# seung-lab/crackle

Measured on AMD Instinct MI355X. Metric: voxels/s encode+decode, 1024x1024x512 uint32; bit-exact .ckl bytes, higher is better.
Workload: dtype u32

## Files before the change

crackle_amd/csrc/ckl_trail.hpp:

```cpp
#pragma once

#include "ckl_device.hpp"

namespace ckl {
namespace dev {

constexpr uint32_t kTrailTileShift = 5, kTrailTileDim = 32;
__device__ __forceinline__ uint32_t mt_index(uint32_t mx, uint32_t my, uint32_t mtx2) {
	return (((my >> 1) * mtx2 + (mx >> 1)) << 2) | ((my & 1u) << 1) | (mx & 1u);
}
struct MicroTile {
	uint4 lo, hi;
	uint32_t mx, my;
	__device__ __forceinline__ bool holds(uint32_t x, uint32_t y) const { return (x >> 3) == mx && (y >> 3) == my; }
	__device__ __forceinline__ uint32_t nib(uint32_t x, uint32_t y) const {
		const uint32_t r = y & 7u;
		const uint32_t a0 = (r & 1u) ? lo.y : lo.x, a1 = (r & 1u) ? lo.w : lo.z, a2 = (r & 1u) ? hi.y : hi.x, a3 = (r & 1u) ? hi.w : hi.z;
		const uint32_t b0 = (r & 2u) ? a1 : a0, b1 = (r & 2u) ? a3 : a2;
		return (((r & 4u) ? b1 : b0) >> ((x & 7u) * 4u)) & 15u;
	}
};

enum : uint32_t { TRAIL_ERR_CAPACITY = 1u };
constexpr uint32_t kDartNone = 0xFFFFFFFFu;
constexpr uint32_t kItemSeg = 0u << 30, kItemCtl = 1u << 30, kItemDead = 2u << 30, kItemMask = 3u << 30;

struct TrailArgs {
	const uint4* adjm;
	uint64_t adjm_stride;
	uint32_t mtx2;
	uint32_t tiles_x, tiles_y;
	const uint32_t* planeV;
	const uint32_t* planeH;
	uint32_t row_words;
	uint64_t plane_words;
	uint32_t sx, sy, inv;
	uint32_t sxe, sye;
	uint32_t nverts;
	uint32_t z0;
	const uint32_t* max_steps;
	uint32_t graph_blocks;
	const uint32_t* blk_special;
	const uint32_t* blk_corner;
	const uint64_t* nbase;
	const uint32_t* ncap;
	uint32_t* n_nodes;
	uint32_t* node_vertex;
	uint8_t* node_adj;
	uint32_t* vert2node;
	const uint64_t* cobase;
	const uint32_t* cocap;
	uint32_t* n_corners;
	uint32_t* corner_vertex;
	uint32_t* dart_end;
	uint32_t* dart_len;
	uint32_t* dart_minv;
	uint32_t* dart_minpos;
	uint4* dart_codes;
	uint8_t* dart_inline;
	uint32_t* parent;
	unsigned long long* compmin;
	uint32_t* start_bits;
	uint32_t start_words;
	uint32_t* starts;
	uint32_t* n_starts;
	const uint64_t* ibase;
	const uint32_t* icap;
	uint32_t* items;
	uint32_t* item_off;
	uint32_t* n_items;
	const uint64_t* sbase;
	const uint32_t* scap;
	uint32_t* stack_node;
	uint32_t* stack_item;
	const uint64_t* kbase;
	const uint32_t* kcap;
	uint32_t* chain_node;
	uint32_t* chain_item0;
	uint32_t* chain_off;
	uint32_t* chain_clen;
	uint32_t* n_chains;
	uint32_t* n_raw;
	uint32_t* n_valid;
	const uint64_t* cbase;
	const uint32_t* ccap;
	uint8_t* cp;
	uint32_t* slice_err;
	uint32_t* events;
	uint32_t* n_events;
	uint32_t* seg_len_sum;
	uint32_t* chain_ev0;
	uint32_t* ev_lnd;
	uint32_t* ev_item;
	uint32_t walk_plain;
	uint32_t walk_stack_cap;
	uint32_t walk_no_regs;
	unsigned long long* dbg;
};

__device__ __forceinline__ void mt_load(MicroTile& c, const uint4* adjm, uint32_t x, uint32_t y, uint32_t mtx2) {
	const uint4* p = adjm + static_cast<uint64_t>(mt_index(x >> 3, y >> 3, mtx2)) * 2u;
	c.lo = p[0]; c.hi = p[1];
	c.mx = x >> 3; c.my = y >> 3;
}
__device__ __forceinline__ void trail_step(uint32_t& x, uint32_t& y, uint32_t k) {
	if (k & 2u) y = (k & 1u) ? y - 1u : y + 1u;
	else x = (k & 1u) ? x - 1u : x + 1u;
}
__device__ __forceinline__ uint32_t trail_code(uint32_t k) { return (0x0231u >> (4u * k)) & 3u; }

struct TileRowBits { uint32_t R, L, D, U; };

__device__ __forceinline__ TileRowBits trail_row_bits(
	const uint32_t* __restrict__ pv, const uint32_t* __restrict__ ph, uint32_t row_words,
	uint32_t sx, uint32_t sy, uint32_t tx, uint32_t y, uint32_t inv
) {
	const uint32_t x0 = tx << 5;
	const uint32_t lt_sx = x0 >= sx ? 0u : (sx - x0 >= 32u ? 0xFFFFFFFFu : ((1u << (sx - x0)) - 1u));
	const uint32_t le_sx = x0 > sx ? 0u : (sx - x0 >= 31u ? 0xFFFFFFFFu : ((2u << (sx - x0)) - 1u));
	const uint32_t ge_1 = tx == 0 ? 0xFFFFFFFEu : 0xFFFFFFFFu;
	TileRowBits b = { 0, 0, 0, 0 };
	const bool have_w = tx < row_words;
	if (y >= 1 && y < sy) {
		const uint32_t h = have_w ? ph[static_cast<uint64_t>(y) * row_words + tx] : 0u;
		const uint32_t hp = tx > 0 ? ph[static_cast<uint64_t>(y) * row_words + tx - 1] : 0u;
		b.R = (h ^ inv) & lt_sx;
		b.L = (((h << 1) | (hp >> 31)) ^ inv) & ge_1 & le_sx;
	}
	if (y < sy) b.D = ((have_w ? pv[static_cast<uint64_t>(y) * row_words + tx] : 0u) ^ inv) & ge_1 & lt_sx;
	if (y >= 1 && y <= sy) b.U = ((have_w ? pv[static_cast<uint64_t>(y - 1) * row_words + tx] : 0u) ^ inv) & ge_1 & lt_sx;
	return b;
}
__device__ __forceinline__ uint32_t trail_special_mask(const TileRowBits& b) {
	const uint32_t a1 = b.R ^ b.L, a2 = b.R & b.L, c1 = b.D ^ b.U, c2 = b.D & b.U;
	const uint32_t bit0 = a1 ^ c1, carry = a1 & c1;
	const uint32_t bit1 = a2 ^ c2 ^ carry, bit2 = (a2 & c2) | (carry & (a2 ^ c2));
	const uint32_t deg2 = ~bit0 & bit1 & ~bit2;
	return (b.R | b.L | b.D | b.U) & ~deg2;
}
__device__ __forceinline__ uint32_t trail_corner_mask(const TileRowBits& b) { return b.R & b.D & ~b.L & ~b.U; }
__device__ __forceinline__ uint32_t spread8(uint32_t m) {
	uint32_t x = (m | (m << 12)) & 0x000F000Fu;
	x = (x | (x << 6)) & 0x03030303u;
	x = (x | (x << 3)) & 0x11111111u;
	return x;
}

__device__ __forceinline__ void trail_rows8(
	const uint32_t* __restrict__ pv, const uint32_t* __restrict__ ph, uint32_t row_words,
	uint32_t sx, uint32_t sy, uint32_t tx, uint32_t y0, uint32_t inv, TileRowBits (&b)[8]
) {
#pragma unroll
	for (int k = 0; k < 8; k++) b[k] = TileRowBits{ 0, 0, 0, 0 };
	if (row_words == 0 || sy == 0) return;
	const uint32_t x0 = tx << 5;
	const uint32_t lt_sx = x0 >= sx ? 0u : (sx - x0 >= 32u ? 0xFFFFFFFFu : ((1u << (sx - x0)) - 1u));
	const uint32_t le_sx = x0 > sx ? 0u : (sx - x0 >= 31u ? 0xFFFFFFFFu : ((2u << (sx - x0)) - 1u));
	const uint32_t ge_1 = tx == 0 ? 0xFFFFFFFEu : 0xFFFFFFFFu;
	const bool have_w = tx < row_words;
	const uint32_t txc = have_w ? tx : row_words - 1u, txp = tx > 0 ? min(tx - 1u, row_words - 1u) : 0u;
	uint32_t hw[8], hpw[8], vw[9];
#pragma unroll
	for (uint32_t k = 0; k < 8; k++) {
		const uint64_t row = static_cast<uint64_t>(min(y0 + k, sy - 1u)) * row_words;
		hw[k] = ph[row + txc];
		hpw[k] = ph[row + txp];
	}
#pragma unroll
	for (uint32_t k = 0; k < 9; k++) {
		const uint32_t y = y0 + k;
		vw[k] = pv[static_cast<uint64_t>(min(y > 0 ? y - 1u : 0u, sy - 1u)) * row_words + txc];
	}
#pragma unroll
	for (uint32_t k = 0; k < 8; k++) {
		const uint32_t y = y0 + k;
		const uint32_t h = have_w ? hw[k] : 0u, hp = tx > 0 ? hpw[k] : 0u;
		if (y >= 1 && y < sy) {
			b[k].R = (h ^ inv) & lt_sx;
			b[k].L = (((h << 1) | (hp >> 31)) ^ inv) & ge_1 & le_sx;
		}
		if (y < sy) b[k].D = ((have_w ? vw[k + 1] : 0u) ^ inv) & ge_1 & lt_sx;
		if (y >= 1 && y <= sy) b[k].U = ((have_w ? vw[k] : 0u) ^ inv) & ge_1 & lt_sx;
	}
}

static __global__ void __launch_bounds__(kBlock) k_trail_graph(
	const uint32_t* __restrict__ planeV, const uint32_t* __restrict__ planeH, uint32_t row_words, uint64_t plane_words,
	uint32_t sx, uint32_t sy, uint32_t perm_mode, const unsigned long long* __restrict__ total_pairs, unsigned long long half_voxels,
	uint32_t* __restrict__ adjm_words, uint64_t adjm_stride_words,
	uint32_t mtx2, uint32_t tiles_x, uint32_t tiles_y, uint32_t* __restrict__ blk_special, uint32_t* __restrict__ blk_corner
) {
	__shared__ uint32_t s_red[2 * kWaves];
	__shared__ uint4 s_out[kWaves][kWave * 8];
	const int lane = threadIdx.x & 63, wave = threadIdx.x >> 6;
	const uint32_t zi = blockIdx.y;
	const bool permissible = perm_mode == 2u ? static_cast<long long>(*total_pairs) < static_cast<long long>(half_voxels) : perm_mode != 0u;
	const uint32_t item = blockIdx.x * kBlock + threadIdx.x;
	const uint32_t mtx = (sx + 1u + 7u) >> 3;
	uint32_t ns = 0, nc = 0;
	uint32_t my_base = 0, my_tiles = 0;
	if (item < tiles_x * tiles_y) {
		const uint32_t ty = item / tiles_x, tx = item - ty * tiles_x;
		TileRowBits b[8];
		trail_rows8(planeV + zi * plane_words, planeH + zi * plane_words, row_words, sx, sy, tx, ty << 3, permissible ? 0xFFFFFFFFu : 0u, b);
		my_base = mt_index(tx * 4u, ty, mtx2) * 32u;
		my_tiles = min(4u, mtx - min(mtx, tx * 4u));
#pragma unroll
		for (uint32_t q = 0; q < 4; q++) {
			uint32_t w[8];
#pragma unroll
			for (uint32_t k = 0; k < 8; k++)
				w[k] = spread8((b[k].R >> (8 * q)) & 255u) | (spread8((b[k].L >> (8 * q)) & 255u) << 1)
					| (spread8((b[k].D >> (8 * q)) & 255u) << 2) | (spread8((b[k].U >> (8 * q)) & 255u) << 3);
			s_out[wave][lane * 8 + ((2u * q) ^ (lane & 7))] = make_uint4(w[0], w[1], w[2], w[3]);
			s_out[wave][lane * 8 + ((2u * q + 1u) ^ (lane & 7))] = make_uint4(w[4], w[5], w[6], w[7]);
		}
#pragma unroll
		for (uint32_t k = 0; k < 8; k++) { ns += __popc(trail_special_mask(b[k])); nc += __popc(trail_corner_mask(b[k])); }
	}
	{
		uint8_t* dst = reinterpret_cast<uint8_t*>(adjm_words + zi * adjm_stride_words);
#pragma unroll
		for (uint32_t i = 0; i < 8; i++) {
			const uint32_t owner = i * 8u + (lane >> 3), p = lane & 7u;
			const uint32_t base = __shfl(my_base, owner, kWave), have = __shfl(my_tiles, owner, kWave);
			const uint4 v = s_out[wave][owner * 8u + (p ^ (owner & 7u))];
			const uint32_t q = p >> 1;
			if (q < have) *reinterpret_cast<uint4*>(dst + base + (q >> 1) * 128u + (q & 1u) * 32u + (p & 1u) * 16u) = v;
		}
	}
	ns = wave_sum(ns); nc = wave_sum(nc);
	if (lane == 0) { s_red[wave] = ns; s_red[kWaves + wave] = nc; }
	__syncthreads();
	if (threadIdx.x == 0) {
		uint32_t ts = 0, tc = 0;
		for (int w = 0; w < kWaves; w++) { ts += s_red[w]; tc += s_red[kWaves + w]; }
		blk_special[static_cast<uint64_t>(zi) * gridDim.x + blockIdx.x] = ts;
		blk_corner[static_cast<uint64_t>(zi) * gridDim.x + blockIdx.x] = tc;
	}
}

static __global__ void __launch_bounds__(kBlock) k_trail_count_scan(
	uint32_t* __restrict__ blk_special, uint32_t* __restrict__ blk_corner, uint32_t nblk,
	uint32_t* __restrict__ tot_special, uint32_t* __restrict__ tot_corner
) {
	__shared__ uint32_t s_scan[2 * kWaves];
	const uint32_t zi = blockIdx.x;
	uint32_t* bs = blk_special + static_cast<uint64_t>(zi) * nblk;
	uint32_t* bc = blk_corner + static_cast<uint64_t>(zi) * nblk;
	uint32_t cs = 0, cc = 0;
	for (uint32_t b0 = 0; b0 < nblk; b0 += kBlock) {
		const uint32_t b = b0 + threadIdx.x;
		uint32_t v[2] = { b < nblk ? bs[b] : 0u, b < nblk ? bc[b] : 0u }, tot[2];
		block_excl_add<2>(v, tot, s_scan);
		if (b < nblk) { bs[b] = cs + v[0]; bc[b] = cc + v[1]; }
		cs += tot[0]; cc += tot[1];
	}
	if (threadIdx.x == 0) { tot_special[zi] = cs; tot_corner[zi] = cc; }
}

static __global__ void __launch_bounds__(kBlock) k_trail_nodes(TrailArgs a) {
	__shared__ uint32_t s_scan[2 * kWaves];
	const uint32_t zi = blockIdx.y + a.z0;
	const uint32_t item = blockIdx.x * kBlock + threadIdx.x;
	TileRowBits b[8];
	uint32_t x0 = 0, y0 = 0;
	if (item < a.tiles_x * a.tiles_y) {
		const uint32_t ty = item / a.tiles_x, tx = item - ty * a.tiles_x;
		x0 = tx << kTrailTileShift; y0 = ty << 3;
		trail_rows8(a.planeV + zi * a.plane_words, a.planeH + zi * a.plane_words, a.row_words, a.sx, a.sy, tx, y0, a.inv, b);
	}
	else {
#pragma unroll
		for (int k = 0; k < 8; k++) b[k] = TileRowBits{ 0, 0, 0, 0 };
	}
	uint32_t v[2] = { 0, 0 }, tot[2];
#pragma unroll
	for (uint32_t k = 0; k < 8; k++) { v[0] += __popc(trail_special_mask(b[k])); v[1] += __popc(trail_corner_mask(b[k])); }
	block_excl_add<2>(v, tot, s_scan);
	uint32_t j = a.blk_special[static_cast<uint64_t>(zi) * a.graph_blocks + blockIdx.x] + v[0];
	uint32_t c = a.blk_corner[static_cast<uint64_t>(zi) * a.graph_blocks + blockIdx.x] + v[1];
	const uint64_t nb = a.nbase[zi];
	const uint32_t ncap = a.ncap[zi], cocap = a.cocap[zi];
	uint32_t err = 0;
#pragma unroll
	for (uint32_t k = 0; k < 8; k++) {
		const uint32_t y = y0 + k;
		const TileRowBits& r = b[k];
		for (uint32_t m = trail_special_mask(r); m; m &= m - 1u) {
			const uint32_t i = __ffs(m) - 1;
			const uint32_t vtx = y * a.sxe + x0 + i;
			if (j < ncap) {
				a.node_vertex[nb + j] = vtx;
				a.node_adj[nb + j] = static_cast<uint8_t>(((r.R >> i) & 1u) | (((r.L >> i) & 1u) << 1) | (((r.D >> i) & 1u) << 2) | (((r.U >> i) & 1u) << 3));
				a.vert2node[static_cast<uint64_t>(zi) * a.nverts + vtx] = j;
			}
			else err = TRAIL_ERR_CAPACITY;
			j++;
		}
		for (uint32_t m = trail_corner_mask(r); m; m &= m - 1u) {
			const uint32_t i = __ffs(m) - 1;
			if (c < cocap) a.corner_vertex[a.cobase[zi] + c] = y * a.sxe + x0 + i;
			else err = TRAIL_ERR_CAPACITY;
			c++;
		}
	}
	if (err) atomicOr(a.slice_err + zi, err);
	if (blockIdx.x == gridDim.x - 1 && threadIdx.x == kBlock - 1) {
		a.n_nodes[zi] = min(j, ncap);
		a.n_corners[zi] = min(c, cocap);
	}
}

constexpr uint32_t kWalkChunk = 192;
constexpr uint32_t kExpandChunk = 384;
constexpr int kWalkRefill = 8;
constexpr int kWalkAhead = 2;
constexpr uint32_t kInlineCodes = 64;

static __global__ void __launch_bounds__(kBlock) k_trail_segments(TrailArgs a) {
	__shared__ uint4 s_res[kWaves][kWalkChunk];
	__shared__ uint4 s_codes[kWaves][kWalkChunk];
	const uint32_t zi = blockIdx.y + a.z0;
	const uint32_t lane = threadIdx.x & (kWave - 1);
	const uint32_t wv = threadIdx.x >> 6;
	const uint32_t wave = blockIdx.x * kWaves + wv;
	const uint32_t n_darts = min(a.n_nodes[zi], a.ncap[zi]) * 4u;
	const uint32_t range_begin = wave * kWalkChunk;
	uint32_t next = range_begin;
	const uint32_t range_end = min(next + kWalkChunk, n_darts);
	if (next >= range_end) return;
	const uint64_t nb = a.nbase[zi];
	const uint4* adjm = a.adjm + zi * a.adjm_stride;
	const uint32_t* v2n = a.vert2node + static_cast<uint64_t>(zi) * a.nverts;
	const uint32_t cap = a.max_steps[zi];
	const unsigned long long lt_mask = (1ull << lane) - 1ull;
	uint4* res = s_res[wv];
	uint4* res_codes = s_codes[wv];
	for (uint32_t i = lane; i < kWalkChunk; i += kWave) res[i] = make_uint4(kDartNone, 0u, 0u, 0u);
	MicroTile c;
	c.lo = c.hi = make_uint4(0, 0, 0, 0); c.mx = c.my = 0xFFFFFFFFu;
	bool active = false;
	uint32_t d = 0, x = 0, y = 0, k = 0, steps = 0, minv = 0, minpos = 0, err = 0;
	uint4 cq = make_uint4(0, 0, 0, 0);
	auto push_code = [&](uint32_t kk) {
		cq.x = __builtin_amdgcn_alignbit(cq.y, cq.x, 2);
		cq.y = __builtin_amdgcn_alignbit(cq.z, cq.y, 2);
		cq.z = __builtin_amdgcn_alignbit(cq.w, cq.z, 2);
		cq.w = (cq.w >> 2) | (trail_code(kk) << 30);
	};
	unsigned long long dbg_iter = 0, dbg_lane = 0;
	const unsigned long long dbg_t0 = a.dbg ? __builtin_amdgcn_s_memtime() : 0ull;
	for (;;) {
		if (a.dbg) { dbg_iter++; dbg_lane += __popcll(__ballot(active)); }
		const unsigned long long need = __ballot(!active);
		const bool refill = next < range_end && (__popcll(need) >= kWalkRefill || need == ~0ull);
		const uint32_t cand = next + static_cast<uint32_t>(__popcll(need & lt_mask));
		const bool take = refill && !active && cand < range_end;
		uint32_t r_adj = 0, r_v0 = 0;
		if (take) { r_adj = a.node_adj[nb + (cand >> 2)]; r_v0 = a.node_vertex[nb + (cand >> 2)]; }
		if (active && !c.holds(x, y)) mt_load(c, adjm, x, y, a.mtx2);
		for (int it = 0; it < kWalkAhead; it++) {
			const bool go = active && c.holds(x, y);
			if (!__ballot(go)) break;
			if (go) {
				const uint32_t w = y * a.sxe + x;
				const uint32_t arr = k ^ 1u;
				if (w < minv) { minv = w; minpos = (steps << 2) | arr; }
				const uint32_t nib = c.nib(x, y);
				bool fin = false;
				if (__popc(nib) != 2) fin = true;
				else if (steps >= cap) { err = TRAIL_ERR_CAPACITY; fin = true; }
				else { k = __ffs(nib & ~(1u << arr)) - 1; push_code(k); trail_step(x, y, k); steps++; }
				if (fin) {
					res[d - range_begin] = make_uint4((w << 2) | arr, steps, minv, minpos);
					res_codes[d - range_begin] = cq;
					active = false;
				}
			}
		}
		if (take && ((r_adj >> (cand & 3u)) & 1u)) {
			d = cand; k = cand & 3u;
			y = r_v0 / a.sxe; x = r_v0 - y * a.sxe;
			minv = r_v0; minpos = 0;
			push_code(k);
			trail_step(x, y, k);
			steps = 1;
			active = true;
		}
		if (refill) next += static_cast<uint32_t>(__popcll(need));
		if (!__ballot(active) && next >= range_end) break;
	}
	if (a.dbg && lane == 0) {
		const unsigned long long cyc = __builtin_amdgcn_s_memtime() - dbg_t0;
		atomicAdd(a.dbg + 0, dbg_iter); atomicMax(a.dbg + 1, dbg_iter);
		atomicAdd(a.dbg + 2, cyc); atomicMax(a.dbg + 3, cyc);
		atomicAdd(a.dbg + 4, 1ull); atomicAdd(a.dbg + 5, dbg_lane);
	}
	const uint64_t db = nb * 4u + range_begin;
	uint32_t len_sum = 0;
	for (uint32_t i = lane; i < range_end - range_begin; i += kWave) {
		const uint4 r = res[i];
		a.dart_end[db + i] = r.x == kDartNone ? kDartNone : ((v2n[r.x >> 2] << 2) | (r.x & 3u));
		a.dart_len[db + i] = r.y;
		a.dart_minv[db + i] = r.z;
		a.dart_minpos[db + i] = r.w;
		const uint4 q = res_codes[i];
		const bool whole = r.x != kDartNone && r.y >= 1u && r.y <= kInlineCodes;
		uint4 o = make_uint4(0, 0, 0, 0);
		if (whole) {
			const uint32_t sh = 128u - 2u * r.y, w = sh >> 5, b = sh & 31u;
			const uint32_t v[5] = { q.x, q.y, q.z, q.w, 0u };
			auto word = [&](uint32_t t) -> uint32_t { return t == 0 ? v[0] : t == 1 ? v[1] : t == 2 ? v[2] : t == 3 ? v[3] : 0u; };
			auto pick = [&](uint32_t t) -> uint32_t { return __builtin_amdgcn_alignbit(word(t + w + 1u), word(t + w), b); };
			o = make_uint4(pick(0), pick(1), pick(2), pick(3));
			(void)v;
		}
		a.dart_codes[db + i] = o;
		a.dart_inline[db + i] = whole ? 1u : 0u;
		len_sum += r.x == kDartNone ? 0u : r.y;
	}
	len_sum = wave_sum(len_sum);
	if (lane == 0 && len_sum) atomicAdd(a.seg_len_sum + zi, len_sum);
	if (err) atomicOr(a.slice_err + zi, err);
}

static __global__ void __launch_bounds__(kBlock) k_trail_loops(TrailArgs a) {
	const uint32_t zi = blockIdx.y + a.z0;
	if (a.seg_len_sum[zi] == 2u * (a.max_steps[zi] - 1u)) return;
	const uint32_t ci = blockIdx.x * kBlock + threadIdx.x;
	const uint32_t nc = min(a.n_corners[zi], a.cocap[zi]);
	const uint4* adjm = a.adjm + zi * a.adjm_stride;
	const uint32_t cap = a.max_steps[zi];
	bool active = ci < nc;
	const uint32_t v0 = active ? a.corner_vertex[a.cobase[zi] + ci] : 0u;
	uint32_t y = v0 / a.sxe, x = v0 - y * a.sxe;
	uint32_t k = 0, steps = 1;
	trail_step(x, y, k);
	bool loop = false;
	MicroTile c;
	c.lo = c.hi = make_uint4(0, 0, 0, 0); c.mx = c.my = 0xFFFFFFFFu;
	while (__ballot(active)) {
		if (active && !c.holds(x, y)) mt_load(c, adjm, x, y, a.mtx2);
		for (int it = 0; it < kWalkAhead; it++) {
			const bool go = active && c.holds(x, y);
			if (!__ballot(go)) break;
			if (go) {
				const uint32_t w = y * a.sxe + x;
				const uint32_t nib = c.nib(x, y);
				if (w == v0) { loop = true; active = false; }
				else if (w < v0 || __popc(nib) != 2 || steps >= cap) active = false;
				else { k = __ffs(nib & ~(1u << (k ^ 1u))) - 1; trail_step(x, y, k); steps++; }
			}
		}
	}
	if (!loop) return;
	const uint32_t j = atomicAdd(a.n_nodes + zi, 1u);
	if (j >= a.ncap[zi]) { atomicOr(a.slice_err + zi, TRAIL_ERR_CAPACITY); return; }
	const uint64_t nb = a.nbase[zi];
	a.node_vertex[nb + j] = v0;
	a.node_adj[nb + j] = 5u;
	a.vert2node[static_cast<uint64_t>(zi) * a.nverts + v0] = j;
	const uint64_t db = (nb + j) * 4u;
	for (uint32_t q = 0; q < 4; q++) { a.dart_end[db + q] = kDartNone; a.dart_len[db + q] = 0; a.dart_minv[db + q] = v0; a.dart_minpos[db + q] = 0; a.dart_inline[db + q] = 0; }
	a.dart_end[db + 0] = (j << 2) | 2u; a.dart_len[db + 0] = steps;
	a.dart_end[db + 2] = (j << 2) | 0u; a.dart_len[db + 2] = steps;
}

template <bool LDS>
__device__ __forceinline__ uint32_t tuf_load(uint32_t* L, uint32_t i) {
	if (LDS) return __hip_atomic_load(L + i, __ATOMIC_RELAXED, __HIP_MEMORY_SCOPE_WORKGROUP);
	return __hip_atomic_load(L + i, __ATOMIC_RELAXED, __HIP_MEMORY_SCOPE_AGENT);
}
template <bool LDS>
__device__ __forceinline__ uint32_t tuf_find(uint32_t* L, uint32_t a) {
	uint32_t p = tuf_load<LDS>(L, a);
	while (p != a) {
		const uint32_t gp = tuf_load<LDS>(L, p);
		if (gp != p) atomicMin(L + a, gp);
		a = p;
		p = gp;
	}
	return a;
}
template <bool LDS>
__device__ __forceinline__ void tuf_unite(uint32_t* L, uint32_t a, uint32_t b) {
	for (;;) {
		a = tuf_find<LDS>(L, a);
		b = tuf_find<LDS>(L, b);
		if (a == b) return;
		if (a > b) { const uint32_t t = a; a = b; b = t; }
		const uint32_t old = atomicMin(L + b, a);
		if (old == b) return;
		b = old;
	}
}

constexpr uint32_t kStartList = 2048;
constexpr int kCompBlock = 256;

template <bool LDS>
__device__ __forceinline__ void trail_components_slice(const TrailArgs& a, uint32_t zi, uint32_t* parent, uint32_t nn, uint32_t* s_scan, uint32_t* s_nstart) {
	const uint64_t nb = a.nbase[zi];
	uint32_t* start_tmp = a.items + a.ibase[zi];
	unsigned long long dg_t = a.dbg ? __builtin_amdgcn_s_memtime() : 0ull;
	auto stamp = [&](int slot) { if (a.dbg && threadIdx.x == 0) { const unsigned long long now = __builtin_amdgcn_s_memtime(); atomicAdd(a.dbg + slot, now - dg_t); dg_t = now; } };
	const uint32_t* dart_end = a.dart_end + nb * 4u;
	unsigned long long* compmin = a.compmin + nb;
	for (uint32_t j = threadIdx.x; j < nn; j += kCompBlock) { parent[j] = j; compmin[j] = ~0ull; }
	__syncthreads();
	if (!LDS) __threadfence();
	constexpr uint32_t kUniteBatch = 8;
	for (uint32_t d0 = threadIdx.x; d0 < nn * 4u; d0 += kCompBlock * kUniteBatch) {
		uint32_t e[kUniteBatch];
#pragma unroll
		for (uint32_t k = 0; k < kUniteBatch; k++) {
			const uint32_t d = d0 + k * kCompBlock;
			e[k] = d < nn * 4u ? dart_end[d] : kDartNone;
		}
#pragma unroll
		for (uint32_t k = 0; k < kUniteBatch; k++) {
			if (e[k] == kDartNone) continue;
			const uint32_t j = (d0 + k * kCompBlock) >> 2, j2 = e[k] >> 2;
			if (j < j2 && j2 < nn) tuf_unite<LDS>(parent, j, j2);
		}
	}
	__syncthreads();
	if (!LDS) __threadfence();
	stamp(12);
	for (uint32_t j0 = 0; j0 < nn; j0 += kCompBlock) {
		const uint32_t j = j0 + threadIdx.x;
		uint32_t root = 0xFFFFFFFFu;
		unsigned long long val = ~0ull;
		if (j < nn) {
			const uint4 e4 = *reinterpret_cast<const uint4*>(dart_end + j * 4u);
			const uint4 m4 = *reinterpret_cast<const uint4*>(a.dart_minv + nb * 4u + j * 4u);
			const uint32_t ee[4] = { e4.x, e4.y, e4.z, e4.w }, mm[4] = { m4.x, m4.y, m4.z, m4.w };
#pragma unroll
			for (uint32_t k = 0; k < 4u; k++) {
				if (ee[k] == kDartNone) continue;
				const unsigned long long v = (static_cast<unsigned long long>(mm[k]) << 32) | (j * 4u + k);
				val = v < val ? v : val;
			}
			if (val != ~0ull) root = tuf_find<LDS>(parent, j);
		}
		unsigned long long todo = __ballot(root != 0xFFFFFFFFu);
		while (todo) {
			const int first = __ffsll(static_cast<long long>(todo)) - 1;
			const uint32_t r0 = __shfl(root, first, kWave);
			const bool mine = (root == r0);
			unsigned long long v = mine ? val : ~0ull;
#pragma unroll
			for (int s = kWave / 2; s >= 1; s >>= 1) {
				const unsigned long long o = __shfl_xor(v, s, kWave);
				v = o < v ? o : v;
			}
			if ((threadIdx.x & (kWave - 1)) == first) atomicMin(compmin + r0, v);
			todo &= ~__ballot(mine);
		}
	}
	__syncthreads();
	__threadfence();
	stamp(13);
	uint32_t* bits = a.start_bits + static_cast<uint64_t>(zi) * a.start_words;
	for (uint32_t j = threadIdx.x; j < nn; j += kCompBlock) {
		if (tuf_load<LDS>(parent, j) != j) continue;
		const unsigned long long m = __hip_atomic_load(compmin + j, __ATOMIC_RELAXED, __HIP_MEMORY_SCOPE_AGENT);
		if (m == ~0ull) continue;
		const uint32_t minv = static_cast<uint32_t>(m >> 32);
		const uint32_t d = static_cast<uint32_t>(m);
		atomicOr(bits + (minv >> 5), 1u << (minv & 31u));
		{
			const uint32_t slot = atomicAdd(s_nstart, 1u);
			if (slot < kStartList) start_tmp[slot] = minv;
		}
		const uint64_t db = nb * 4u;
		const uint32_t len = a.dart_len[db + d];
		const uint32_t pos = a.dart_minpos[db + d] >> 2, arr = a.dart_minpos[db + d] & 3u;
		if (pos == 0 || pos == len) continue;
		const uint32_t s = atomicAdd(a.n_nodes + zi, 1u);
		if (s >= a.ncap[zi]) { atomicOr(a.slice_err + zi, TRAIL_ERR_CAPACITY); continue; }
		a.node_vertex[nb + s] = minv;
		a.node_adj[nb + s] = 5u;
		a.vert2node[static_cast<uint64_t>(zi) * a.nverts + minv] = s;
		const uint32_t d2 = a.dart_end[db + d];
		const uint32_t other = arr ^ 2u;
		for (uint32_t q = 0; q < 4; q++) { a.dart_end[db + s * 4u + q] = kDartNone; a.dart_len[db + s * 4u + q] = 0; a.dart_inline[db + s * 4u + q] = 0; }
		a.dart_end[db + d] = (s << 2) | arr;        a.dart_len[db + d] = pos;
		a.dart_end[db + d2] = (s << 2) | other;     a.dart_len[db + d2] = len - pos;
		a.dart_end[db + s * 4u + arr] = d;          a.dart_len[db + s * 4u + arr] = pos;
		a.dart_end[db + s * 4u + other] = d2;       a.dart_len[db + s * 4u + other] = len - pos;
	}
	__syncthreads();
	__threadfence();
	stamp(14);
	uint32_t* starts = a.starts + nb;
	const uint32_t cap = a.kcap[zi];
	const uint32_t n_listed = *s_nstart;
	if (n_listed <= kStartList) {
		for (uint32_t i = threadIdx.x; i < n_listed; i += kCompBlock) {
			const uint32_t v = __hip_atomic_load(start_tmp + i, __ATOMIC_RELAXED, __HIP_MEMORY_SCOPE_AGENT);
			uint32_t rank = 0;
			for (uint32_t q = 0; q < n_listed; q++) rank += __hip_atomic_load(start_tmp + q, __ATOMIC_RELAXED, __HIP_MEMORY_SCOPE_AGENT) < v ? 1u : 0u;
			if (rank < cap) starts[rank] = v;
			else atomicOr(a.slice_err + zi, TRAIL_ERR_CAPACITY);
		}
		if (threadIdx.x == 0) a.n_starts[zi] = n_listed < cap ? n_listed : cap;
		stamp(15);
		return;
	}
	constexpr uint32_t kPer = 8;
	uint32_t carry = 0, err = 0;
	for (uint32_t w0 = 0; w0 < a.start_words; w0 += kCompBlock * kPer) {
		uint32_t b[kPer], cnt = 0;
#pragma unroll
		for (uint32_t q = 0; q < kPer; q++) {
			const uint32_t wi = w0 + threadIdx.x * kPer + q;
			b[q] = wi < a.start_words ? __hip_atomic_load(bits + wi, __ATOMIC_RELAXED, __HIP_MEMORY_SCOPE_AGENT) : 0u;
			cnt += __popc(b[q]);
		}
		uint32_t v[1] = { cnt }, tot[1];
		block_excl_add<1, kCompBlock / kWave>(v, tot, s_scan);
		uint32_t o = carry + v[0];
#pragma unroll
		for (uint32_t q = 0; q < kPer; q++) {
			const uint32_t wi = w0 + threadIdx.x * kPer + q;
			for (uint32_t m = b[q]; m; m &= m - 1u) {
				if (o < cap) starts[o] = wi * 32u + (__ffs(m) - 1);
				else err = TRAIL_ERR_CAPACITY;
				o++;
			}
		}
		carry += tot[0];
	}
	if (threadIdx.x == 0) a.n_starts[zi] = carry < cap ? carry : cap;
	if (err) atomicOr(a.slice_err + zi, err);
	stamp(15);
}

static __global__ void __launch_bounds__(kCompBlock) k_trail_components(TrailArgs a, uint32_t lds_bytes) {
	extern __shared__ uint32_t s_trail[];
	__shared__ uint32_t s_scan[kCompBlock / kWave];
	__shared__ uint32_t s_nstart;
	const uint32_t zi = blockIdx.x + a.z0;
	const uint32_t nn = min(a.n_nodes[zi], a.ncap[zi]);
	if (threadIdx.x == 0) s_nstart = 0;
	__syncthreads();
	if (nn * 4u <= lds_bytes) trail_components_slice<true>(a, zi, s_trail, nn, s_scan, &s_nstart);
	else trail_components_slice<false>(a, zi, a.parent + a.nbase[zi], nn, s_scan, &s_nstart);
}

enum : uint32_t { TCODE_UP = 0, TCODE_RIGHT = 1, TCODE_DOWN = 2, TCODE_LEFT = 3, TCODE_NONE = 0xFE };

struct TrailTabLds {
	uint8_t* adj;
	unsigned long long* end4;
	__device__ __forceinline__ void load(uint32_t j, uint32_t& av, uint32_t& e_lo, uint32_t& e_hi) const {
		const uint32_t a0 = adj[j];
		const unsigned long long e = end4[j];
		av = __builtin_amdgcn_readfirstlane(a0);
		e_lo = __builtin_amdgcn_readfirstlane(static_cast<uint32_t>(e));
		e_hi = __builtin_amdgcn_readfirstlane(static_cast<uint32_t>(e >> 32));
	}
	__device__ __forceinline__ uint32_t pick(uint32_t e_lo, uint32_t e_hi, uint32_t k) const {
		const uint32_t w = (k & 2u) ? e_hi : e_lo;
		return (w >> ((k & 1u) * 16u)) & 0xFFFFu;
	}
	__device__ __forceinline__ void set_adj(uint32_t j, uint32_t v) const { adj[j] = static_cast<uint8_t>(v); }
};
struct TrailTabGlobal {
	uint8_t* adj;
	const uint32_t* end;
	__device__ __forceinline__ void load(uint32_t j, uint32_t& av, uint32_t& e_lo, uint32_t& e_hi) const {
		const uint32_t* w = reinterpret_cast<const uint32_t*>(reinterpret_cast<uintptr_t>(adj + j) & ~static_cast<uintptr_t>(3));
		const uint32_t sh = static_cast<uint32_t>(reinterpret_cast<uintptr_t>(adj + j) & 3u) * 8u;
		av = (__builtin_amdgcn_readfirstlane(__hip_atomic_load(w, __ATOMIC_RELAXED, __HIP_MEMORY_SCOPE_AGENT)) >> sh) & 0xFFu;
		e_lo = j; e_hi = 0;
	}
	__device__ __forceinline__ uint32_t pick(uint32_t e_lo, uint32_t e_hi, uint32_t k) const { return __builtin_amdgcn_readfirstlane(end[e_lo * 4u + k]); }
	__device__ __forceinline__ void set_adj(uint32_t j, uint32_t v) const {
		uint32_t* w = reinterpret_cast<uint32_t*>(reinterpret_cast<uintptr_t>(adj + j) & ~static_cast<uintptr_t>(3));
		const uint32_t sh = static_cast<uint32_t>(reinterpret_cast<uintptr_t>(adj + j) & 3u) * 8u;
		const uint32_t old = __hip_atomic_load(w, __ATOMIC_RELAXED, __HIP_MEMORY_SCOPE_AGENT);
		__hip_atomic_store(w, (old & ~(0xFFu << sh)) | ((v & 0xFFu) << sh), __ATOMIC_RELAXED, __HIP_MEMORY_SCOPE_AGENT);
	}
};

constexpr uint32_t kEvSeg = 0u << 30, kEvBseg = 1u << 30, kEvDead = 2u << 30, kEvEnd = 3u << 30, kEvMask = 3u << 30;
constexpr uint32_t kEvFormatAddr12 = 1u << 31;
constexpr uint32_t kEvWalkWide = 1u << 30;

template <typename TAB>
__device__ __forceinline__ void trail_walk_slice(
	const TrailArgs& a, uint32_t zi, const TAB& tab, uint2* s_stack2, uint32_t lds_slots
) {
	const uint64_t nb = a.nbase[zi];
	const uint32_t* starts = a.starts + nb;
	const uint32_t n_starts = a.n_starts[zi];
	uint32_t* ev = a.events + a.ibase[zi];
	const uint32_t ecap = a.icap[zi];
	uint32_t* st_node = a.stack_node + a.sbase[zi];
	uint32_t* st_ev = a.stack_item + a.sbase[zi];
	const uint32_t scap = a.scap[zi];
	uint32_t* ch_node = a.chain_node + a.kbase[zi];
	uint32_t* ch_ev0 = a.chain_ev0 + a.kbase[zi];
	const uint32_t kcap = a.kcap[zi];
	const uint32_t* vert2node = a.vert2node + static_cast<uint64_t>(zi) * a.nverts;
	const uint32_t cap1 = lds_slots - 1u;

	uint32_t ne = 0, nch = 0, err = 0;
	const unsigned long long dbg_t0 = (kTuning && a.dbg) ? __builtin_amdgcn_s_memtime() : 0ull;
	const unsigned long long dbg_r0 = (kTuning && a.dbg) ? __builtin_amdgcn_s_memrealtime() : 0ull;
	for (uint32_t si = 0; si < n_starts && !err; si++) {
		const uint32_t sv = __builtin_amdgcn_readfirstlane(starts[si]);
		uint32_t j = __builtin_amdgcn_readfirstlane(vert2node[sv]);
		if (nch < kcap) { ch_node[nch] = sv; ch_ev0[nch] = ne; }
		else err |= TRAIL_ERR_CAPACITY;
		nch++;
		uint32_t sp = 0, pend = 0;
		for (;;) {
			if (ne + 2u > ecap) { err |= TRAIL_ERR_CAPACITY; break; }
			uint32_t av_raw, e_lo, e_hi;
			tab.load(j, av_raw, e_lo, e_hi);
// ... 935 lines not shown
```

Baseline: 151.5 billion.

## Pack trail walker coordinates and cache micro-tiles in LDS per lane

Rewrites the segment-walking kernel so each lane tracks position as a packed y<<xb|x word. Moving becomes a single add driven by bitfield lookup tables, which replaces separate x/y updates and the per-step y*sxe multiply. The current adjacency micro-tile is copied into a per-lane shared-memory buffer and the nibble is read with one LDS load, instead of register select chains. Results are stored structure-of-arrays, the walk chunk shrinks to 128, and refill uses mbcnt. This adds LDS pressure that may reduce occupancy, and it converts packed coordinates back to linear form at output.

```diff
diff --git a/crackle_amd/csrc/ckl_trail.hpp b/crackle_amd/csrc/ckl_trail.hpp
--- a/crackle_amd/csrc/ckl_trail.hpp
+++ b/crackle_amd/csrc/ckl_trail.hpp
@@ -109,6 +109,8 @@
 }
 __device__ __forceinline__ uint32_t trail_code(uint32_t k) { return (0x0231u >> (4u * k)) & 3u; }
 
+__device__ __forceinline__ uint32_t trail_xbits(uint32_t sx) { return min(29u, 32u - static_cast<uint32_t>(__builtin_clz(sx | 15u))); }
+
 struct TileRowBits { uint32_t R, L, D, U; };
 
 __device__ __forceinline__ TileRowBits trail_row_bits(
@@ -312,15 +314,22 @@
 	}
 }
 
-constexpr uint32_t kWalkChunk = 192;
+constexpr uint32_t kWalkChunk = 128;
 constexpr uint32_t kExpandChunk = 384;
 constexpr int kWalkRefill = 8;
 constexpr int kWalkAhead = 2;
+constexpr int kSegRefill = 8;
+constexpr int kSegAhead = 2;
+constexpr uint32_t kSegTileXBits = 3, kSegTileYBits = 3;
+static_assert(kSegTileXBits == 3 || kSegTileXBits == 4, "");
+static_assert(kSegTileYBits == 3 || (kSegTileYBits == 4 && kSegTileXBits == 4), "micro-tiles that follow each other in memory");
+constexpr uint32_t kSegTiles = 1u << (kSegTileXBits + kSegTileYBits - 6), kSegTileRows = 8u * kSegTiles;
 constexpr uint32_t kInlineCodes = 64;
 
 static __global__ void __launch_bounds__(kBlock) k_trail_segments(TrailArgs a) {
-	__shared__ uint4 s_res[kWaves][kWalkChunk];
+	__shared__ uint32_t s_res[kWaves][4][kWalkChunk];
 	__shared__ uint4 s_codes[kWaves][kWalkChunk];
+	__shared__ uint32_t s_tile[kWaves][kSegTileRows][kWave];
 	const uint32_t zi = blockIdx.y + a.z0;
 	const uint32_t lane = threadIdx.x & (kWave - 1);
 	const uint32_t wv = threadIdx.x >> 6;
@@ -334,46 +343,69 @@
 	const uint4* adjm = a.adjm + zi * a.adjm_stride;
 	const uint32_t* v2n = a.vert2node + static_cast<uint64_t>(zi) * a.nverts;
 	const uint32_t cap = a.max_steps[zi];
-	const unsigned long long lt_mask = (1ull << lane) - 1ull;
-	uint4* res = s_res[wv];
+	const uint32_t xb = trail_xbits(a.sx), xmask = (1u << xb) - 1u;
+	const uint32_t tile_mask = ~(((1u << kSegTileXBits) - 1u) | (((1u << kSegTileYBits) - 1u) << xb));
+	const uint32_t k_shift = (xb << 16) | (xb << 24);
+	constexpr uint32_t k_sign = 0xFF01FF01u;
+	constexpr uint32_t k_code = 0x00020301u;
+	uint32_t* res = &s_res[wv][0][0];
 	uint4* res_codes = s_codes[wv];
-	for (uint32_t i = lane; i < kWalkChunk; i += kWave) res[i] = make_uint4(kDartNone, 0u, 0u, 0u);
-	MicroTile c;
-	c.lo = c.hi = make_uint4(0, 0, 0, 0); c.mx = c.my = 0xFFFFFFFFu;
+	uint32_t* tl = &s_tile[wv][0][lane];
+	for (uint32_t i = lane; i < kWalkChunk; i += kWave) res[kWalkChunk + i] = 0u;
 	bool active = false;
-	uint32_t d = 0, x = 0, y = 0, k = 0, steps = 0, minv = 0, minpos = 0, err = 0;
+	uint32_t tile = 0xFFFFFFFFu;
+	uint32_t d = 0, yx = 0, k = 0, steps = 0, minv = 0, minpos = 0, err = 0;
 	uint4 cq = make_uint4(0, 0, 0, 0);
-	auto push_code = [&](uint32_t kk) {
+	auto move = [&](uint32_t kk) {
+		const uint32_t k8 = kk << 3;
 		cq.x = __builtin_amdgcn_alignbit(cq.y, cq.x, 2);
 		cq.y = __builtin_amdgcn_alignbit(cq.z, cq.y, 2);
 		cq.z = __builtin_amdgcn_alignbit(cq.w, cq.z, 2);
-		cq.w = (cq.w >> 2) | (trail_code(kk) << 30);
+		cq.w = __builtin_amdgcn_alignbit(__builtin_amdgcn_ubfe(k_code, k8, 2u), cq.w, 2);
+		yx += static_cast<uint32_t>(__builtin_amdgcn_sbfe(static_cast<int>(k_sign), k8, 8u)) << __builtin_amdgcn_ubfe(k_shift, k8, 8u);
 	};
 	unsigned long long dbg_iter = 0, dbg_lane = 0;
 	const unsigned long long dbg_t0 = a.dbg ? __builtin_amdgcn_s_memtime() : 0ull;
 	for (;;) {
-		if (a.dbg) { dbg_iter++; dbg_lane += __popcll(__ballot(active)); }
-		const unsigned long long need = __ballot(!active);
-		const bool refill = next < range_end && (__popcll(need) >= kWalkRefill || need == ~0ull);
-		const uint32_t cand = next + static_cast<uint32_t>(__popcll(need & lt_mask));
-		const bool take = refill && !active && cand < range_end;
-		uint32_t r_adj = 0, r_v0 = 0;
-		if (take) { r_adj = a.node_adj[nb + (cand >> 2)]; r_v0 = a.node_vertex[nb + (cand >> 2)]; }
-		if (active && !c.holds(x, y)) mt_load(c, adjm, x, y, a.mtx2);
-		for (int it = 0; it < kWalkAhead; it++) {
-			const bool go = active && c.holds(x, y);
-			if (!__ballot(go)) break;
+		if (a.dbg) { dbg_iter++; dbg_lane += __popcll(__builtin_amdgcn_ballot_w64(active)); }
+		const unsigned long long need = __builtin_amdgcn_ballot_w64(!active);
+		const uint32_t n_need = static_cast<uint32_t>(__popcll(need));
+		bool take = false;
+		uint32_t cand = 0, r_adj = 0, r_v0 = 0;
+		if (next < range_end && (n_need >= static_cast<uint32_t>(kSegRefill) || need == ~0ull)) {
+			cand = next + __builtin_amdgcn_mbcnt_hi(static_cast<uint32_t>(need >> 32), __builtin_amdgcn_mbcnt_lo(static_cast<uint32_t>(need), 0u));
+			take = !active && cand < range_end;
+			if (take) { r_adj = a.node_adj[nb + (cand >> 2)]; r_v0 = a.node_vertex[nb + (cand >> 2)]; }
+			next += n_need;
+		}
+		if (active && (yx & tile_mask) != tile) {
+			const uint32_t mx = ((yx & xmask) >> kSegTileXBits) << (kSegTileXBits - 3u), my = ((yx >> xb) >> kSegTileYBits) << (kSegTileYBits - 3u);
+			const uint4* p = adjm + static_cast<uint64_t>(mt_index(mx, my, a.mtx2)) * 2u;
+			uint4 q[2 * kSegTiles];
+#pragma unroll
+			for (uint32_t t = 0; t < 2u * kSegTiles; t++) q[t] = p[t];
+#pragma unroll
+			for (uint32_t t = 0; t < kSegTiles; t++) {
+				uint32_t* o = tl + (((t >> 1) * 8u + ((t & 1u) << kSegTileYBits)) * kWave);
+				o[0 * kWave] = q[2 * t].x; o[1 * kWave] = q[2 * t].y; o[2 * kWave] = q[2 * t].z; o[3 * kWave] = q[2 * t].w;
+				o[4 * kWave] = q[2 * t + 1].x; o[5 * kWave] = q[2 * t + 1].y; o[6 * kWave] = q[2 * t + 1].z; o[7 * kWave] = q[2 * t + 1].w;
+			}
+			tile = yx & tile_mask;
+		}
+		for (int it = 0; it < kSegAhead; it++) {
+			const bool go = active && (yx & tile_mask) == tile;
+			if (!__builtin_amdgcn_ballot_w64(go)) break;
 			if (go) {
-				const uint32_t w = y * a.sxe + x;
 				const uint32_t arr = k ^ 1u;
-				if (w < minv) { minv = w; minpos = (steps << 2) | arr; }
-				const uint32_t nib = c.nib(x, y);
-				bool fin = false;
-				if (__popc(nib) != 2) fin = true;
-				else if (steps >= cap) { err = TRAIL_ERR_CAPACITY; fin = true; }
-				else { k = __ffs(nib & ~(1u << arr)) - 1; push_code(k); trail_step(x, y, k); steps++; }
-				if (fin) {
-					res[d - range_begin] = make_uint4((w << 2) | arr, steps, minv, minpos);
+				if (yx < minv) { minv = yx; minpos = (steps << 2) | arr; }
+				const uint32_t row = __builtin_amdgcn_ubfe(yx, xb, kSegTileYBits) | (kSegTileXBits == 4 ? (yx & 8u) << (kSegTileYBits - 3u) : 0u);
+				const uint32_t nib = __builtin_amdgcn_ubfe(tl[row * kWave], (yx & 7u) << 2, 4u);
+				const bool through = __popc(nib) == 2;
+				if (through && steps < cap) { k = __ffs(nib & ~(1u << arr)) - 1; move(k); steps++; }
+				else {
+					if (through) err = TRAIL_ERR_CAPACITY;
+					uint32_t* r = res + (d - range_begin);
+					r[0] = yx; r[kWalkChunk] = (steps << 2) | arr; r[2 * kWalkChunk] = minv; r[3 * kWalkChunk] = minpos;
 					res_codes[d - range_begin] = cq;
 					active = false;
 				}
@@ -381,15 +413,13 @@
 		}
 		if (take && ((r_adj >> (cand & 3u)) & 1u)) {
 			d = cand; k = cand & 3u;
-			y = r_v0 / a.sxe; x = r_v0 - y * a.sxe;
-			minv = r_v0; minpos = 0;
-			push_code(k);
-			trail_step(x, y, k);
+			const uint32_t y0 = r_v0 / a.sxe;
+			yx = minv = (y0 << xb) | (r_v0 - y0 * a.sxe); minpos = 0;
+			move(k);
 			steps = 1;
 			active = true;
 		}
-		if (refill) next += static_cast<uint32_t>(__popcll(need));
-		if (!__ballot(active) && next >= range_end) break;
+		if (!__builtin_amdgcn_ballot_w64(active) && next >= range_end) break;
 	}
 	if (a.dbg && lane == 0) {
 		const unsigned long long cyc = __builtin_amdgcn_s_memtime() - dbg_t0;
@@ -400,25 +430,26 @@
 	const uint64_t db = nb * 4u + range_begin;
 	uint32_t len_sum = 0;
 	for (uint32_t i = lane; i < range_end - range_begin; i += kWave) {
-		const uint4 r = res[i];
-		a.dart_end[db + i] = r.x == kDartNone ? kDartNone : ((v2n[r.x >> 2] << 2) | (r.x & 3u));
-		a.dart_len[db + i] = r.y;
-		a.dart_minv[db + i] = r.z;
+		const uint4 r = make_uint4(res[i], res[kWalkChunk + i], res[2 * kWalkChunk + i], res[3 * kWalkChunk + i]);
+		const bool none = r.y == 0u;
+		const uint32_t len = r.y >> 2;
+		const uint32_t wend = (r.x >> xb) * a.sxe + (r.x & xmask);
+		a.dart_end[db + i] = none ? kDartNone : ((v2n[wend] << 2) | (r.y & 3u));
+		a.dart_len[db + i] = len;
+		a.dart_minv[db + i] = (r.z >> xb) * a.sxe + (r.z & xmask);
 		a.dart_minpos[db + i] = r.w;
 		const uint4 q = res_codes[i];
-		const bool whole = r.x != kDartNone && r.y >= 1u && r.y <= kInlineCodes;
+		const bool whole = len >= 1u && len <= kInlineCodes;
 		uint4 o = make_uint4(0, 0, 0, 0);
 		if (whole) {
-			const uint32_t sh = 128u - 2u * r.y, w = sh >> 5, b = sh & 31u;
-			const uint32_t v[5] = { q.x, q.y, q.z, q.w, 0u };
-			auto word = [&](uint32_t t) -> uint32_t { return t == 0 ? v[0] : t == 1 ? v[1] : t == 2 ? v[2] : t == 3 ? v[3] : 0u; };
+			const uint32_t sh = 128u - 2u * len, w = sh >> 5, b = sh & 31u;
+			auto word = [&](uint32_t t) -> uint32_t { return t == 0 ? q.x : t == 1 ? q.y : t == 2 ? q.z : t == 3 ? q.w : 0u; };
 			auto pick = [&](uint32_t t) -> uint32_t { return __builtin_amdgcn_alignbit(word(t + w + 1u), word(t + w), b); };
 			o = make_uint4(pick(0), pick(1), pick(2), pick(3));
-			(void)v;
 		}
 		a.dart_codes[db + i] = o;
 		a.dart_inline[db + i] = whole ? 1u : 0u;
-		len_sum += r.x == kDartNone ? 0u : r.y;
+		len_sum += len;
 	}
 	len_sum = wave_sum(len_sum);
 	if (lane == 0 && len_sum) atomicAdd(a.seg_len_sum + zi, len_sum);
```

Measured after the change: 150.0 billion. -1.0%, worse.
